# vnoz/Mutual-Information-MultiModal

Measured on AMD Instinct MI355X. Metric: img-txt pairs/sec (MI critic fwd+bwd), global-batch InfoNCE, higher is better.
Workload: dtype bf16; 1 GPU; BASELINE configs[3]: global-batch infonce (reference semantics), bilinear critic fwd+bwd, B_global=4096, d=512; global_batch=4096, embed_dim=512, critic=bilinear, estimator=infonce, parallelism=single GPU, boundary=fp32 embeddings in, fp32 gradients out, hip_graph=False, graph_mode=none (direct C-ABI calls)

## Files before the change

### mutual-information-multimodal_amd/csrc/mi_bilinear_tail.h

```cpp
#pragma once
#include "mi_bilinear_flash.h"

namespace mi {

struct FlashTailArgs {
  FlashReduceJob j[2];
  const mi_stats* stats;
  const float* grad_out;
  const Partial* merge_rec;
  int64_t n_merge, n_pos;
  int estimator;
  float* loss_out;
  mi_stats* stats_out;
  float* partials_out;
  const bf16_t* w_frag;
  int64_t dx;
  float* grad_x;
  bf16_t* grad_x_bf;
  bf16_t* dtt_frag;
  int n_blocks0;
  const bf16_t* w_frag1;
  int64_t dx1;
  float* grad_x1;
  bf16_t* dtt_frag1;
};

#ifndef MI_TAIL_REC_FIRST
#define MI_TAIL_REC_FIRST 1
#endif
constexpr int kTailPad = 4;
constexpr int kTailThreads = 512;

template <int D, bool F16, bool MERGE, bool GBF = false>
__global__ __launch_bounds__(kTailThreads, 2) void flash_tail_kernel(FlashTailArgs args) {
  kernarg_prefetch<(int)sizeof(FlashTailArgs)>();
  MI_WALL_SCOPE(kWallTail);
  extern __shared__ __attribute__((aligned(16))) char smem_tail[];
  float(*tile)[D + kTailPad] = reinterpret_cast<float(*)[D + kTailPad]>(smem_tail);
  const int tid = threadIdx.x, lane = tid & 63, wave = __builtin_amdgcn_readfirstlane(tid >> 6);
  const int blk = (int)blockIdx.x;
  const int job = blk >= args.n_blocks0 ? 1 : 0;
  const FlashReduceJob& J = args.j[job];
  const int64_t wb = job ? blk - args.n_blocks0 : blk;
  if (wb * 32 >= J.m) return;
  const int rb = (int)(wb >> 2), w = (int)(wb & 3);
  const int64_t i0 = wb * 32;
  const f16_t* slab16 = reinterpret_cast<const f16_t*>(J.slab);
  const float* unscale = reinterpret_cast<const float*>(slab16 + (int64_t)J.n_split * J.n_rb * 4 * (32 * D));
  constexpr int NC = D / 128;

  int64_t wvs[4];
#pragma unroll
  for (int q = 0; q < 4; ++q) wvs[q] = ((int64_t)(q < J.n_split ? q : J.n_split - 1) * J.n_rb + rb) * 4 + w;

  Partial pre[2];
  float m_rec[4], u_rec[4], go_pre;
  auto load_heads = [&]() __attribute__((always_inline)) {
    if constexpr (MERGE) {
#pragma unroll
      for (int u = 0; u < 2; ++u) {
        const int64_t k = tid + 256 * u;
        pre[u] = args.merge_rec[k < args.n_merge ? k : args.n_merge - 1];
      }
    }
#pragma unroll
    for (int q = 0; q < 4; ++q) {
      m_rec[q] = J.rec[wvs[q]].m;
      u_rec[q] = F16 ? unscale[wvs[q]] : 1.0f;
    }
    go_pre = *(args.grad_out ? args.grad_out : &J.rec[wvs[0]].m);
  };
  if constexpr (MI_TAIL_REC_FIRST) load_heads();

  f16x8 vh[NC][4];
  f32x4 vf[NC][4][2];
#pragma unroll
  for (int cc = 0; cc < NC; ++cc)
#pragma unroll
    for (int q = 0; q < 4; ++q) {
      if constexpr (F16) {
        vh[cc][q] = *reinterpret_cast<const f16x8*>(slab16 + wvs[q] * (32 * D) + (int64_t)cc * 4096 + tid * 8);
      } else {
#pragma unroll
        for (int u = 0; u < 2; ++u)
          vf[cc][q][u] = *reinterpret_cast<const f32x4*>(J.slab + wvs[q] * (32 * D) + (int64_t)cc * 4096 + (u * 512 + tid) * 4);
      }
    }

  if constexpr (!MI_TAIL_REC_FIRST) load_heads();

  const int orow = tid >> 4;
  const int64_t ojo = i0 + orow + J.diag;
  const bool has_other = ojo >= 0 && ojo < J.n_other;
  const int64_t ojc = has_other ? ojo : 0;
  bf16x8 oth[D / 128];
#pragma unroll
  for (int g = 0; g < D / 128; ++g) oth[g] = *reinterpret_cast<const bf16x8*>(J.other + ojc * D + ((tid & 15) + 16 * g) * 8);

  float lse, n_pos_f;
  if constexpr (MERGE) {
    char* extra = smem_tail + (size_t)32 * (D + kTailPad) * sizeof(float);
    Partial* scratch = reinterpret_cast<Partial*>(extra);
    unsigned long long* cnt_scratch = reinterpret_cast<unsigned long long*>(extra + 64);
    float& lse_sh = *reinterpret_cast<float*>(extra + 96);
    if (wave < 4) {
      Partial p{MI_NEG_INF, 0.0f, 0.0f, 0u};
      unsigned long long cnt = 0;
#pragma unroll
      for (int u = 0; u < 2; ++u)
        if (tid + 256 * u < args.n_merge) {
          lse_merge(p.m, p.s, pre[u].m, pre[u].s);
          p.pos += pre[u].pos;
          cnt += pre[u].cnt;
        }
      for (int64_t k = tid + 512; k < args.n_merge; k += 256) {
        const Partial q = args.merge_rec[k];
        lse_merge(p.m, p.s, q.m, q.s);
        p.pos += q.pos;
        cnt += q.cnt;
      }
      for (int o = 32; o > 0; o >>= 1) cnt += __shfl_xor(cnt, o);
      wave_lse(p.m, p.s);
      p.pos = wave_sum(p.pos);
      if (lane == 0) {
        cnt_scratch[wave] = cnt;
        p.cnt = 0;
        scratch[wave] = p;
      }
    }
    __syncthreads();
    if (tid == 0) {
      Partial p = scratch[0];
      for (int k = 1; k < 4; ++k) {
        lse_merge(p.m, p.s, scratch[k].m, scratch[k].s);
        p.pos += scratch[k].pos;
      }
      const unsigned long long total = cnt_scratch[0] + cnt_scratch[1] + cnt_scratch[2] + cnt_scratch[3];
      const float l = (p.s > 0.0f) ? p.m + logf(p.s) : MI_NEG_INF;
      lse_sh = l;
      if (blk == 0) {
        if (args.partials_out) {
          float* r = args.partials_out;
          r[0] = p.m; r[1] = p.s; r[2] = p.pos;
          r[3] = (float)(total & 0xFFFFFFull); r[4] = (float)(total >> 24);
          r[5] = r[6] = r[7] = 0.0f;
        }
        mi_stats* st = args.stats_out;
        const float pos_mean = p.pos / (float)args.n_pos;
        const float log_n = logf((float)total);
        st->lse = l; st->pos_mean = pos_mean; st->log_n_neg = log_n; st->neg_max = p.m;
        st->loss_dv = (l - log_n) - pos_mean;
        st->loss_infonce = l - pos_mean;
        st->reserved0 = st->reserved1 = 0.0f;
        st->n_neg = (int64_t)total; st->n_pos = args.n_pos; st->reserved2 = st->reserved3 = 0;
        if (args.loss_out) args.loss_out[0] = (args.estimator == MI_DV) ? st->loss_dv : st->loss_infonce;
      }
    }
    __syncthreads();
    lse = lse_sh;
    n_pos_f = (float)args.n_pos;
  } else {
    lse = args.stats->lse;
    n_pos_f = (float)args.stats->n_pos;
  }
  const float go = args.grad_out ? go_pre : 1.0f;
  const float gpos = go / n_pos_f;

  float cs[4];
  for (int s0 = 0; s0 < J.n_split; s0 += 4) {
#pragma unroll
    for (int q = 0; q < 4; ++q) {
      const int s = s0 + q < J.n_split ? s0 + q : J.n_split - 1;
      wvs[q] = ((int64_t)s * J.n_rb + rb) * 4 + w;
      if (s0 > 0) {
        m_rec[q] = J.rec[wvs[q]].m;
        u_rec[q] = F16 ? unscale[wvs[q]] : 1.0f;
      }
      cs[q] = (s0 + q < J.n_split && m_rec[q] > MI_NEG_INF) ? go * __expf(m_rec[q] - lse) * u_rec[q] : 0.0f;
    }
    if (s0 > 0) {
#pragma unroll
      for (int cc = 0; cc < NC; ++cc)
#pragma unroll
        for (int q = 0; q < 4; ++q) {
          if constexpr (F16) {
            vh[cc][q] = *reinterpret_cast<const f16x8*>(slab16 + wvs[q] * (32 * D) + (int64_t)cc * 4096 + tid * 8);
          } else {
#pragma unroll
            for (int u = 0; u < 2; ++u)
              vf[cc][q][u] = *reinterpret_cast<const f32x4*>(J.slab + wvs[q] * (32 * D) + (int64_t)cc * 4096 + (u * 512 + tid) * 4);
          }
        }
    }
#pragma unroll
    for (int cc = 0; cc < NC; ++cc) {
      if constexpr (F16) {
        float acc[8];
#pragma unroll
        for (int e = 0; e < 8; ++e) acc[e] = 0.0f;
#pragma unroll
        for (int q = 0; q < 4; ++q)
          if (cs[q] != 0.0f) {
#pragma unroll
            for (int e = 0; e < 8; ++e) acc[e] += (float)vh[cc][q][e] * cs[q];
          }
        const int ct_l = tid >> 7, gp = (tid >> 6) & 1, ln = tid & 63;
        const int col = cc * 128 + ct_l * 32 + (ln & 31);
#pragma unroll
        for (int hh = 0; hh < 2; ++hh) {
          const int row0 = 8 * (2 * gp + hh) + 4 * (ln >> 5);
#pragma unroll
          for (int e = 0; e < 4; ++e) {
            if (s0 == 0) tile[row0 + e][col] = acc[4 * hh + e];
            else tile[row0 + e][col] += acc[4 * hh + e];
          }
        }
      } else {
        float acc[8];
#pragma unroll
        for (int e = 0; e < 8; ++e) acc[e] = 0.0f;
#pragma unroll
        for (int q = 0; q < 4; ++q)
          if (cs[q] != 0.0f) {
#pragma unroll
            for (int u = 0; u < 2; ++u)
#pragma unroll
              for (int e = 0; e < 4; ++e) acc[4 * u + e] += vf[cc][q][u][e] * cs[q];
          }
#pragma unroll
        for (int u = 0; u < 2; ++u) {
          const int f = u * 512 + tid;
          const int ct_l = f >> 8, g = (f >> 6) & 3, ln = f & 63;
          const int col = cc * 128 + ct_l * 32 + (ln & 31), row0 = 8 * g + 4 * (ln >> 5);
#pragma unroll
          for (int e = 0; e < 4; ++e) {
            if (s0 == 0) tile[row0 + e][col] = acc[4 * u + e];
            else tile[row0 + e][col] += acc[4 * u + e];
          }
        }
      }
    }
  }
  __syncthreads();

  {
    const int row = orow;
    const int64_t i = i0 + row;
#pragma unroll
    for (int g = 0; g < D / 128; ++g) {
      const int c = ((tid & 15) + 16 * g) * 8;
      float v[8];
#pragma unroll
      for (int e = 0; e < 8; ++e) v[e] = tile[row][c + e];
      if (has_other) {
        const bf16x8 o = oth[g];
#pragma unroll
        for (int e = 0; e < 8; ++e) v[e] -= gpos * (float)o[e];
        if (job == 0 || args.w_frag1 != nullptr) {
#pragma unroll
          for (int e = 0; e < 8; ++e) tile[row][c + e] = v[e];
        }
      }
      if constexpr (GBF) {
        if (J.out_bf) {
          const bf16x8 o = {(bf16_t)v[0], (bf16_t)v[1], (bf16_t)v[2], (bf16_t)v[3],
                            (bf16_t)v[4], (bf16_t)v[5], (bf16_t)v[6], (bf16_t)v[7]};
          seam_store<kSeam_TAIL_GRAD>(reinterpret_cast<bf16x8*>(J.out_bf + i * D + c), o);
        }
      } else if (J.out_f32) {
        seam_store<kSeam_TAIL_GRAD>(reinterpret_cast<f32x4*>(J.out_f32 + i * D + c), f32x4{v[0], v[1], v[2], v[3]});
        seam_store<kSeam_TAIL_GRAD>(reinterpret_cast<f32x4*>(J.out_f32 + i * D + c + 4), f32x4{v[4], v[5], v[6], v[7]});
      }
    }
  }
  if (job != 0) {
    if (GBF || args.w_frag1 == nullptr) return;
  } else if (GBF ? args.grad_x_bf == nullptr : args.grad_x == nullptr) {
    return;
  }
  const bf16_t* const w_frag = job ? args.w_frag1 : args.w_frag;
  const int64_t dx_out = job ? args.dx1 : args.dx;
  float* const gx_out = job ? args.grad_x1 : args.grad_x;
  bf16_t* const dtt_out = job ? args.dtt_frag1 : args.dtt_frag;
  __syncthreads();

  constexpr int NK = D / 16;
  const int r = lane & 31, h = lane >> 5;
  const int64_t n_at = dx_out / 32;
  constexpr int PF = 8;
  bf16x8 bq[PF][2];
  const bf16_t* wbase[2];
  {
    const int64_t at0 = wave * 2;
#pragma unroll
    for (int t = 0; t < 2; ++t) {
      const int64_t at = at0 + t < n_at ? at0 + t : n_at - 1;
      wbase[t] = w_frag + (at * NK * 64 + lane) * 8;
    }
#pragma unroll
    for (int p = 0; p < PF; ++p)
#pragma unroll
      for (int t = 0; t < 2; ++t) bq[p][t] = *reinterpret_cast<const bf16x8*>(wbase[t] + (int64_t)p * 512);
  }

  {
    const int64_t nkb = J.m / 16;
#pragma unroll
    for (int q = 0; q < (D / 32) * 2 / 8; ++q) {
      const int bi = wave + 8 * q;
      const int cb = bi >> 1, kl = bi & 1;
      bf16x8 o;
#pragma unroll
      for (int jj = 0; jj < 8; ++jj) o[jj] = (bf16_t)tile[16 * kl + 8 * h + jj][32 * cb + r];
      seam_store<kSeam_TAIL_DTT>(reinterpret_cast<bf16x8*>(dtt_out + (((int64_t)cb * nkb + (i0 / 16 + kl)) * 64 + lane) * 8), o);
    }
  }

  for (int64_t at0 = wave * 2; at0 < n_at; at0 += 16) {
    f32x16 acc[2];
#pragma unroll
    for (int t = 0; t < 2; ++t)
#pragma unroll
      for (int e = 0; e < 16; ++e) acc[t][e] = 0.0f;
    if (at0 != wave * 2) {
#pragma unroll
      for (int t = 0; t < 2; ++t) {
        const int64_t at = at0 + t < n_at ? at0 + t : n_at - 1;
        wbase[t] = w_frag + (at * NK * 64 + lane) * 8;
      }
#pragma unroll
      for (int p = 0; p < PF; ++p)
#pragma unroll
        for (int t = 0; t < 2; ++t) bq[p][t] = *reinterpret_cast<const bf16x8*>(wbase[t] + (int64_t)p * 512);
    }
#pragma unroll
    for (int kk = 0; kk < NK; ++kk) {
      const f32x4 a0 = *reinterpret_cast<const f32x4*>(&tile[r][16 * kk + 8 * h]);
      const f32x4 a1 = *reinterpret_cast<const f32x4*>(&tile[r][16 * kk + 8 * h + 4]);
      const bf16x8 af = {(bf16_t)a0[0], (bf16_t)a0[1], (bf16_t)a0[2], (bf16_t)a0[3],
                         (bf16_t)a1[0], (bf16_t)a1[1], (bf16_t)a1[2], (bf16_t)a1[3]};
#pragma unroll
      for (int t = 0; t < 2; ++t) acc[t] = __builtin_amdgcn_mfma_f32_32x32x16_bf16(af, bq[kk % PF][t], acc[t], 0, 0, 0);
      if (kk + PF < NK) {
#pragma unroll
        for (int t = 0; t < 2; ++t) bq[kk % PF][t] = *reinterpret_cast<const bf16x8*>(wbase[t] + (int64_t)(kk + PF) * 512);
      }
    }
#pragma unroll
    for (int t = 0; t < 2; ++t) {
      if (at0 + t >= n_at) continue;
#pragma unroll
      for (int g = 0; g < 4; ++g)
#pragma unroll
        for (int e = 0; e < 4; ++e) {
          const int64_t o = (i0 + 8 * g + 4 * h + e) * dx_out + (at0 + t) * 32 + r;
          if constexpr (GBF) seam_store<kSeam_TAIL_GRAD>(&args.grad_x_bf[o], (bf16_t)acc[t][4 * g + e]);
          else seam_store<kSeam_TAIL_GRAD>(&gx_out[o], acc[t][4 * g + e]);
        }
    }
  }
}

template <int D, bool F16, bool MERGE, bool GBF = false>
static inline int launch_flash_tail_t(const FlashTailArgs& a, unsigned grid, hipStream_t st, const char* what) {
  const size_t smem = (size_t)32 * (D + kTailPad) * sizeof(float) + 128;
  MI_SET_DYN_SMEM((flash_tail_kernel<D, F16, MERGE, GBF>), smem, "hipFuncSetAttribute(flash_tail_kernel)");
  {
    ProfScope prof_(what, st);
    hipLaunchKernelGGL((flash_tail_kernel<D, F16, MERGE, GBF>), dim3(grid), dim3(kTailThreads), smem, st, a);
  }
  MI_LAUNCH_CHECK(what);
  return MI_OK;
}

static inline int launch_flash_tail(FlashTailArgs a, int64_t d, bool slab_f16, bool merge, hipStream_t st, const char* what) {
  a.n_blocks0 = (int)(a.j[0].m / 32);
  for (int k = 0; k < 2; ++k)
    if (a.j[k].m > 0 && (a.j[k].n_other < 1 || a.j[k].other == nullptr)) {
      set_error("launch_flash_tail: job %d has no rows to subtract on the diagonal", k);
      return MI_EINVAL;
    }
  if (merge && (a.n_merge < 1 || a.merge_rec == nullptr)) {
    set_error("launch_flash_tail: the merged form needs at least one record");
    return MI_EINVAL;
  }
  const unsigned grid = (unsigned)(a.n_blocks0 + a.j[1].m / 32);
#define MI_TAIL_CASE(DD)                                                                          \
  if (d == DD) {                                                                                  \
    if (a.grad_x_bf) {   \
      if (!(slab_f16 && merge)) {                                                                 \
        set_error("launch_flash_tail: bf16 gradients need fp16 slabs and the merged form");       \
        return MI_EINVAL;                                                                         \
      }                                                                                           \
      return launch_flash_tail_t<DD, true, true, true>(a, grid, st, what);                        \
    }                                                                                             \
    if (slab_f16) return merge ? launch_flash_tail_t<DD, true, true>(a, grid, st, what)           \
                               : launch_flash_tail_t<DD, true, false>(a, grid, st, what);         \
    return merge ? launch_flash_tail_t<DD, false, true>(a, grid, st, what)                        \
                 : launch_flash_tail_t<DD, false, false>(a, grid, st, what);                      \
  }
  MI_TAIL_CASE(512)
  MI_TAIL_CASE(256)
  MI_TAIL_CASE(128)
#undef MI_TAIL_CASE
  set_error("launch_flash_tail: unsupported width %lld", (long long)d);
  return MI_ESHAPE;
}

struct DwArgs {
  const bf16_t* xt_frag;
  const bf16_t* dtt_frag;
  int64_t dx, dy, k;
  float* out;
};

constexpr int kDwWaves = 8;
struct DwArgs2 {
  DwArgs p[2];
  int n_tiles0;
  int natural;
};
static __global__ __launch_bounds__(64 * kDwWaves, 1) void bilinear_dw_kernel(DwArgs2 a2) {
  __shared__ float part[kDwWaves - 1][32][33];
  MI_WALL_SCOPE(kWallDw);
  const int prob = (int)blockIdx.x >= a2.n_tiles0 ? 1 : 0;
  const DwArgs& a = a2.p[prob];
  const int64_t tile_id = prob ? (int64_t)blockIdx.x - a2.n_tiles0 : (int64_t)blockIdx.x;
  const int tid = threadIdx.x, lane = tid & 63, wave = __builtin_amdgcn_readfirstlane(tid >> 6);
  const int64_t nct = a.dy / 32, nat = a.dx / 32;
  int64_t at = tile_id / nct, ct = tile_id % nct;
  if (!a2.natural && nat % 4 == 0 && nct % 2 == 0 && (prob == 0 || a2.n_tiles0 % 8 == 0)) {
    const int64_t xcd = tile_id & 7, i = tile_id >> 3, br = nat / 4, bc = nct / 2;
    at = br * (xcd >> 1) + i / bc;
    ct = bc * (xcd & 1) + i % bc;
  }
  const int64_t nkb = a.k / 16;
  const int64_t kb0 = nkb * wave / kDwWaves, kb1 = nkb * (wave + 1) / kDwWaves;
  const bf16_t* ap = a.xt_frag + ((at * nkb + kb0) * 64 + lane) * 8;
  const bf16_t* bp = a.dtt_frag + ((ct * nkb + kb0) * 64 + lane) * 8;
  f32x16 acc;
#pragma unroll
  for (int e = 0; e < 16; ++e) acc[e] = 0.0f;
  constexpr int PF = 16;
  bf16x8 af[PF], bfr[PF];
  const int64_t n = kb1 - kb0;
#pragma unroll
  for (int p = 0; p < PF; ++p) {
    const int64_t q = p < n ? p : n - 1;
    af[p] = *reinterpret_cast<const bf16x8*>(ap + q * 512);
    bfr[p] = *reinterpret_cast<const bf16x8*>(bp + q * 512);
  }
  for (int64_t q0 = 0; q0 < n; q0 += PF) {
#pragma unroll
    for (int p = 0; p < PF; ++p) {
      if (q0 + p < n) acc = __builtin_amdgcn_mfma_f32_32x32x16_bf16(af[p], bfr[p], acc, 0, 0, 0);
      const int64_t q = q0 + p + PF;
      if (q < n) {
        af[p] = *reinterpret_cast<const bf16x8*>(ap + q * 512);
        bfr[p] = *reinterpret_cast<const bf16x8*>(bp + q * 512);
      }
    }
  }
  const int r = lane & 31, h = lane >> 5;
  if (wave > 0) {
#pragma unroll
    for (int g = 0; g < 4; ++g)
#pragma unroll
      for (int e = 0; e < 4; ++e) part[wave - 1][8 * g + 4 * h + e][r] = acc[4 * g + e];
  }
  __syncthreads();
  if (wave == 0) {
#pragma unroll
    for (int g = 0; g < 4; ++g)
#pragma unroll
      for (int e = 0; e < 4; ++e) {
        const int row = 8 * g + 4 * h + e;
        float v = acc[4 * g + e];
#pragma unroll
        for (int k = 0; k < kDwWaves - 1; ++k) v += part[k][row][r];
        seam_store<kSeam_DW>(&a.out[(at * 32 + row) * a.dy + ct * 32 + r], v);
      }
  }
}

static inline int launch_bilinear_dw(const DwArgs& a, hipStream_t st, const char* what, const DwArgs* b = nullptr) {
  DwArgs2 a2{};
  a2.p[0] = a;
  a2.p[1] = b ? *b : a;
  a2.n_tiles0 = (int)((a.dx / 32) * (a.dy / 32));
  static const int natural = getenv("MI_DW_XCD_NATURAL") ? 1 : 0;
  a2.natural = natural;
  const unsigned grid = (unsigned)(a2.n_tiles0 + (b ? (b->dx / 32) * (b->dy / 32) : 0));
  {
    ProfScope prof_(what, st);
    hipLaunchKernelGGL(bilinear_dw_kernel, dim3(grid), dim3(64 * kDwWaves), 0, st, a2);
  }
  MI_LAUNCH_CHECK(what);
  return MI_OK;
}

static inline bool flash_tail_ok(int64_t br, int64_t dx, int64_t dy) {
  return br % 128 == 0 && dx % 32 == 0 && dy % 32 == 0 && flash_width_ok(dy);
}

}
```

Baseline: 41.46 million pairs/s.

## Balance flash tail work by splitting grad-x GEMM and job-1 reduce across block pairs

Adds a balanced mapping for the flash tail kernel. Before, blocks of job 0 did both the slab reduce and the grad-x GEMM while job-1 blocks did only the reduce. Now each 32-row block is handled by a pair of blocks: each does half of the grad-x output tiles and half of the job-1 column chunks. The pairing is XCD-aware when n_blocks0 is a multiple of 8. The aim is to remove the load imbalance between the two block types, at the cost of redundant job-0 reduction work and more code complexity. It also adds kernarg prefetch and a by-value select of the args in the dW kernel, so it no longer indexes the kernel arguments dynamically.

```diff
diff --git a/mutual-information-multimodal_amd/csrc/mi_bilinear_tail.h b/mutual-information-multimodal_amd/csrc/mi_bilinear_tail.h
--- a/mutual-information-multimodal_amd/csrc/mi_bilinear_tail.h
+++ b/mutual-information-multimodal_amd/csrc/mi_bilinear_tail.h
@@ -31,17 +31,45 @@
 constexpr int kTailPad = 4;
 constexpr int kTailThreads = 512;
 
-template <int D, bool F16, bool MERGE, bool GBF = false>
+template <int D>
+__device__ __forceinline__ void tail_add_chunk_f16(float (*tile)[D + kTailPad], const f16x8 (&v)[4], const float (&cs)[4],
+                                                   int cc, bool first, int tid) {
+  float acc[8];
+#pragma unroll
+  for (int e = 0; e < 8; ++e) acc[e] = 0.0f;
+#pragma unroll
+  for (int q = 0; q < 4; ++q)
+    if (cs[q] != 0.0f) {
+#pragma unroll
+      for (int e = 0; e < 8; ++e) acc[e] += (float)v[q][e] * cs[q];
+    }
+  const int ct_l = tid >> 7, gp = (tid >> 6) & 1, ln = tid & 63;
+  const int col = cc * 128 + ct_l * 32 + (ln & 31);
+#pragma unroll
+  for (int hh = 0; hh < 2; ++hh) {
+    const int row0 = 8 * (2 * gp + hh) + 4 * (ln >> 5);
+#pragma unroll
+    for (int e = 0; e < 4; ++e) {
+      if (first) tile[row0 + e][col] = acc[4 * hh + e];
+      else tile[row0 + e][col] += acc[4 * hh + e];
+    }
+  }
+}
+
+template <int D, bool F16, bool MERGE, bool GBF = false, bool BAL = false>
 __global__ __launch_bounds__(kTailThreads, 2) void flash_tail_kernel(FlashTailArgs args) {
+  static_assert(!BAL || (F16 && MERGE && !GBF && D == 512), "the balanced mapping: see tail_balanced_ok");
   kernarg_prefetch<(int)sizeof(FlashTailArgs)>();
   MI_WALL_SCOPE(kWallTail);
   extern __shared__ __attribute__((aligned(16))) char smem_tail[];
   float(*tile)[D + kTailPad] = reinterpret_cast<float(*)[D + kTailPad]>(smem_tail);
   const int tid = threadIdx.x, lane = tid & 63, wave = __builtin_amdgcn_readfirstlane(tid >> 6);
   const int blk = (int)blockIdx.x;
-  const int job = blk >= args.n_blocks0 ? 1 : 0;
+  const int job = !BAL && blk >= args.n_blocks0 ? 1 : 0;
+  const int hf = !BAL ? 0 : args.n_blocks0 % 8 == 0 ? (blk >> 3) & 1 : blk & 1;
   const FlashReduceJob& J = args.j[job];
-  const int64_t wb = job ? blk - args.n_blocks0 : blk;
+  const int64_t wb = BAL ? (args.n_blocks0 % 8 == 0 ? (blk & 7) + 8 * (blk >> 4) : blk >> 1)
+                         : job ? blk - args.n_blocks0 : blk;
   if (wb * 32 >= J.m) return;
   const int rb = (int)(wb >> 2), w = (int)(wb & 3);
   const int64_t i0 = wb * 32;
@@ -195,26 +223,7 @@
 #pragma unroll
     for (int cc = 0; cc < NC; ++cc) {
       if constexpr (F16) {
-        float acc[8];
-#pragma unroll
-        for (int e = 0; e < 8; ++e) acc[e] = 0.0f;
-#pragma unroll
-        for (int q = 0; q < 4; ++q)
-          if (cs[q] != 0.0f) {
-#pragma unroll
-            for (int e = 0; e < 8; ++e) acc[e] += (float)vh[cc][q][e] * cs[q];
-          }
-        const int ct_l = tid >> 7, gp = (tid >> 6) & 1, ln = tid & 63;
-        const int col = cc * 128 + ct_l * 32 + (ln & 31);
-#pragma unroll
-        for (int hh = 0; hh < 2; ++hh) {
-          const int row0 = 8 * (2 * gp + hh) + 4 * (ln >> 5);
-#pragma unroll
-          for (int e = 0; e < 4; ++e) {
-            if (s0 == 0) tile[row0 + e][col] = acc[4 * hh + e];
-            else tile[row0 + e][col] += acc[4 * hh + e];
-          }
-        }
+        tail_add_chunk_f16<D>(tile, vh[cc], cs, cc, s0 == 0, tid);
       } else {
         float acc[8];
 #pragma unroll
@@ -272,6 +281,119 @@
         seam_store<kSeam_TAIL_GRAD>(reinterpret_cast<f32x4*>(J.out_f32 + i * D + c + 4), f32x4{v[4], v[5], v[6], v[7]});
       }
     }
+  }
+  if constexpr (BAL) {
+    __syncthreads();
+    constexpr int NK = D / 16, PF = 8, NCH = NC / 2;
+    const int r = lane & 31, h = lane >> 5;
+    const int64_t n_at = args.dx / 32, n_at0 = (n_at + 1) / 2;
+    const int64_t t_lo = hf ? n_at0 : 0, t_hi = hf ? n_at : n_at0;
+    bf16x8 bq[PF];
+    const bf16_t* wbase;
+    auto w_head = [&](int64_t at) __attribute__((always_inline)) {
+      wbase = args.w_frag + ((at < n_at ? at : n_at - 1) * NK * 64 + lane) * 8;
+#pragma unroll
+      for (int p = 0; p < PF; ++p) bq[p] = *reinterpret_cast<const bf16x8*>(wbase + (int64_t)p * 512);
+    };
+    w_head(t_lo + wave);
+
+    const FlashReduceJob& L = args.j[1];
+    const f16_t* lslab = reinterpret_cast<const f16_t*>(L.slab);
+    const float* lunscale = reinterpret_cast<const float*>(lslab + (int64_t)L.n_split * L.n_rb * 4 * (32 * D));
+    const int cc0 = hf * NCH;
+    int64_t lw[4];
+    float lm[4], lu[4];
+    f16x8 lv[NCH][4];
+#pragma unroll
+    for (int q = 0; q < 4; ++q) {
+      lw[q] = ((int64_t)(q < L.n_split ? q : L.n_split - 1) * L.n_rb + rb) * 4 + w;
+      lm[q] = L.rec[lw[q]].m;
+      lu[q] = lunscale[lw[q]];
+    }
+#pragma unroll
+    for (int cc = 0; cc < NCH; ++cc)
+#pragma unroll
+      for (int q = 0; q < 4; ++q)
+        lv[cc][q] = *reinterpret_cast<const f16x8*>(lslab + lw[q] * (32 * D) + (int64_t)(cc0 + cc) * 4096 + tid * 8);
+    const int64_t ljo = i0 + orow + L.diag;
+    const bool l_other = ljo >= 0 && ljo < L.n_other;
+    bf16x8 loth[NCH];
+#pragma unroll
+    for (int g = 0; g < NCH; ++g)
+      loth[g] = *reinterpret_cast<const bf16x8*>(L.other + (l_other ? ljo : 0) * D + ((tid & 15) + 16 * (cc0 + g)) * 8);
+
+    {
+      const int64_t nkb = J.m / 16;
+#pragma unroll
+      for (int q = 0; q < NCH; ++q) {
+        const int bi = wave + 8 * (cc0 + q);
+        const int cb = bi >> 1, kl = bi & 1;
+        bf16x8 o;
+#pragma unroll
+        for (int jj = 0; jj < 8; ++jj) o[jj] = (bf16_t)tile[16 * kl + 8 * h + jj][32 * cb + r];
+        seam_store<kSeam_TAIL_DTT>(reinterpret_cast<bf16x8*>(args.dtt_frag + (((int64_t)cb * nkb + (i0 / 16 + kl)) * 64 + lane) * 8), o);
+      }
+    }
+    for (int64_t at = t_lo + wave; at < t_hi; at += 8) {
+      asm volatile("" ::: "memory");
+      f32x16 acc;
+#pragma unroll
+      for (int e = 0; e < 16; ++e) acc[e] = 0.0f;
+#pragma unroll
+      for (int kk = 0; kk < NK; ++kk) {
+        const f32x4 a0 = *reinterpret_cast<const f32x4*>(&tile[r][16 * kk + 8 * h]);
+        const f32x4 a1 = *reinterpret_cast<const f32x4*>(&tile[r][16 * kk + 8 * h + 4]);
+        const bf16x8 af = {(bf16_t)a0[0], (bf16_t)a0[1], (bf16_t)a0[2], (bf16_t)a0[3],
+                           (bf16_t)a1[0], (bf16_t)a1[1], (bf16_t)a1[2], (bf16_t)a1[3]};
+        acc = __builtin_amdgcn_mfma_f32_32x32x16_bf16(af, bq[kk % PF], acc, 0, 0, 0);
+        if (kk + PF < NK) bq[kk % PF] = *reinterpret_cast<const bf16x8*>(wbase + (int64_t)(kk + PF) * 512);
+      }
+      if (at + 8 < t_hi) w_head(at + 8);
+#pragma unroll
+      for (int g = 0; g < 4; ++g)
+#pragma unroll
+        for (int e = 0; e < 4; ++e)
+          seam_store<kSeam_TAIL_GRAD>(&args.grad_x[(i0 + 8 * g + 4 * h + e) * args.dx + at * 32 + r], acc[4 * g + e]);
+    }
+    __syncthreads();
+
+    for (int s0 = 0; s0 < L.n_split; s0 += 4) {
+#pragma unroll
+      for (int q = 0; q < 4; ++q) {
+        if (s0 > 0) {
+          lw[q] = ((int64_t)(s0 + q < L.n_split ? s0 + q : L.n_split - 1) * L.n_rb + rb) * 4 + w;
+          lm[q] = L.rec[lw[q]].m;
+          lu[q] = lunscale[lw[q]];
+        }
+        cs[q] = (s0 + q < L.n_split && lm[q] > MI_NEG_INF) ? go * __expf(lm[q] - lse) * lu[q] : 0.0f;
+      }
+      if (s0 > 0) {
+#pragma unroll
+        for (int cc = 0; cc < NCH; ++cc)
+#pragma unroll
+          for (int q = 0; q < 4; ++q)
+            lv[cc][q] = *reinterpret_cast<const f16x8*>(lslab + lw[q] * (32 * D) + (int64_t)(cc0 + cc) * 4096 + tid * 8);
+      }
+#pragma unroll
+      for (int cc = 0; cc < NCH; ++cc) tail_add_chunk_f16<D>(tile, lv[cc], cs, cc0 + cc, s0 == 0, tid);
+    }
+    __syncthreads();
+#pragma unroll
+    for (int g = 0; g < NCH; ++g) {
+      const int c = ((tid & 15) + 16 * (cc0 + g)) * 8;
+      float v[8];
+#pragma unroll
+      for (int e = 0; e < 8; ++e) v[e] = tile[orow][c + e];
+      if (l_other) {
+        const bf16x8 o = loth[g];
+#pragma unroll
+        for (int e = 0; e < 8; ++e) v[e] -= gpos * (float)o[e];
+      }
+      float* out = L.out_f32 + (i0 + orow) * D + c;
+      seam_store<kSeam_TAIL_GRAD>(reinterpret_cast<f32x4*>(out), f32x4{v[0], v[1], v[2], v[3]});
+      seam_store<kSeam_TAIL_GRAD>(reinterpret_cast<f32x4*>(out + 4), f32x4{v[4], v[5], v[6], v[7]});
+    }
+    return;
   }
   if (job != 0) {
     if (GBF || args.w_frag1 == nullptr) return;
@@ -361,16 +483,22 @@
   }
 }
 
-template <int D, bool F16, bool MERGE, bool GBF = false>
+template <int D, bool F16, bool MERGE, bool GBF = false, bool BAL = false>
 static inline int launch_flash_tail_t(const FlashTailArgs& a, unsigned grid, hipStream_t st, const char* what) {
   const size_t smem = (size_t)32 * (D + kTailPad) * sizeof(float) + 128;
-  MI_SET_DYN_SMEM((flash_tail_kernel<D, F16, MERGE, GBF>), smem, "hipFuncSetAttribute(flash_tail_kernel)");
+  MI_SET_DYN_SMEM((flash_tail_kernel<D, F16, MERGE, GBF, BAL>), smem, "hipFuncSetAttribute(flash_tail_kernel)");
   {
     ProfScope prof_(what, st);
-    hipLaunchKernelGGL((flash_tail_kernel<D, F16, MERGE, GBF>), dim3(grid), dim3(kTailThreads), smem, st, a);
+    hipLaunchKernelGGL((flash_tail_kernel<D, F16, MERGE, GBF, BAL>), dim3(grid), dim3(kTailThreads), smem, st, a);
   }
   MI_LAUNCH_CHECK(what);
   return MI_OK;
+}
+
+static inline bool tail_balanced_ok(const FlashTailArgs& a, int64_t d, bool slab_f16, bool merge) {
+  static const bool whole = getenv("MI_TAIL_WHOLE_BLOCKS") != nullptr;
+  return !whole && d == 512 && slab_f16 && merge && a.j[0].m == a.j[1].m && a.w_frag1 == nullptr &&
+         a.grad_x != nullptr && a.grad_x_bf == nullptr && a.j[0].out_f32 == nullptr && a.j[1].out_f32 != nullptr;
 }
 
 static inline int launch_flash_tail(FlashTailArgs a, int64_t d, bool slab_f16, bool merge, hipStream_t st, const char* what) {
@@ -385,6 +513,7 @@
     return MI_EINVAL;
   }
   const unsigned grid = (unsigned)(a.n_blocks0 + a.j[1].m / 32);
+  if (tail_balanced_ok(a, d, slab_f16, merge)) return launch_flash_tail_t<512, true, true, false, true>(a, grid, st, what);
 #define MI_TAIL_CASE(DD)                                                                          \
   if (d == DD) {                                                                                  \
     if (a.grad_x_bf) {   \
@@ -421,10 +550,13 @@
   int natural;
 };
 static __global__ __launch_bounds__(64 * kDwWaves, 1) void bilinear_dw_kernel(DwArgs2 a2) {
+  kernarg_prefetch<(int)sizeof(DwArgs2)>();
   __shared__ float part[kDwWaves - 1][32][33];
   MI_WALL_SCOPE(kWallDw);
   const int prob = (int)blockIdx.x >= a2.n_tiles0 ? 1 : 0;
-  const DwArgs& a = a2.p[prob];
+  const DwArgs a = {prob ? a2.p[1].xt_frag : a2.p[0].xt_frag, prob ? a2.p[1].dtt_frag : a2.p[0].dtt_frag,
+                    prob ? a2.p[1].dx : a2.p[0].dx,           prob ? a2.p[1].dy : a2.p[0].dy,
+                    prob ? a2.p[1].k : a2.p[0].k,             prob ? a2.p[1].out : a2.p[0].out};
   const int64_t tile_id = prob ? (int64_t)blockIdx.x - a2.n_tiles0 : (int64_t)blockIdx.x;
   const int tid = threadIdx.x, lane = tid & 63, wave = __builtin_amdgcn_readfirstlane(tid >> 6);
   const int64_t nct = a.dy / 32, nat = a.dx / 32;
```

Result: slower. 40.43 million pairs/s (-2.5%).
